# wenyuqing/panacea

Measured on AMD Instinct MI355X. Metric: denoising steps/s (6-view x 8-frame 256x512), higher is better.
Workload: dtype f16; 1 GPU; BASELINE config 3: Panacea+ stage-2 UNet+ControlNet, CFG 2 x 8 frames, 6 views, latent 32x384, hint 256x3072, Euler/LegacyDDPM 50-step schedule; precision=precise: split(stream,gn_stt,ff_out,stem,gn_head,gnt)+e4m3-lo, parallelism=single, graph=False, streams=2, hoisted_step_invariants=False, fused_step_tail=True

## Files before the change

### include/panacea_hip.h

```cpp
#ifndef PANACEA_HIP_H
#define PANACEA_HIP_H

#include <stdint.h>

#ifdef __cplusplus
extern "C" {
#endif

#define PNC_OK 0
#define PNC_EINVAL (-1)
#define PNC_EALIGN (-2)
#define PNC_EABI (-3)

const char* pnc_version(void);
#define PNC_ABI_VERSION 8
int pnc_abi_version(void);
const char* pnc_build_digest(void);

enum {
    PNC_OPT_GEMM_TAIL_SPLIT = 0,
    PNC_OPT_GEMM_TILE = 1,
    PNC_OPT_ATTN_VARIANT = 2,
    PNC_OPT_ATTN_DMA = 3,
    PNC_OPT_GEMM_FUSE_LN = 4,
    PNC_OPT_GEMM_GROUP_M = 5,
    PNC_OPT_STENCIL_TILES = 6,
    PNC_OPT_GEMM_PERSIST = 7,
    PNC_OPT_ATTN_DEFER_MAX = 8,
    PNC_OPT_GEMM_GN_STATS = 9,
    PNC_OPT_GEMM_STAGGER = 10,
    PNC_OPT_ATTN_SUM_TRIGGER = 11,
    PNC_OPT_COUNT = 12
};
int pnc_set_option(int option, int value);

enum { PNC_A_PLAIN = 0, PNC_A_CONV3X3 = 1, PNC_A_CONV1D_T = 2 };
enum { PNC_LO_F16 = 0, PNC_LO_E4M3 = 1 };
enum { PNC_ACT_NONE = 0, PNC_ACT_SILU = 1, PNC_ACT_GELU = 2  };

typedef struct PncGemmParams {
    const void* A;
    const void* W;
    int32_t M, N, K;
    int32_t lda;
    int32_t a_mode;
    int32_t Cin, Hin, Win, Hout, Wout, stride, upsample;
    int32_t T, Npix;
    const float* bias;
    const float* rowbias;
    int32_t rb_rows, rb_mod;
    const float* res1; int32_t ldr1;
    const float* res2; int32_t ldr2;
    float*  out32;  int32_t ldc32;
    void*   out16;  int32_t ldc16;
    void*   out16t; int32_t ldt; int32_t t_rows; int64_t t_gstride;
    int32_t n_split;
    int32_t act;
    int32_t geglu;
    float*  ws;
    int64_t ws_floats;
    int32_t conv_pad_br;
    int32_t struct_bytes;
    const void* A_lo;
    void* out16_lo;
    int32_t ldw;
    float ln_eps;
    const float* ln_gamma;
    const float* ln_beta;
    void* ln_out16;
    int32_t ldln;
    int32_t a_lo_fmt;
    int32_t out_lo_fmt;
    int32_t ldw_lo;
    const void* W_lo;
    int32_t w_lo_exp;
    int32_t t_halo;
    int64_t x_halo_off;
    float* gn_part;
} PncGemmParams;

int pnc_gemm_f16(const PncGemmParams* p, void* stream);
int pnc_gemm_wsplit_f16(const PncGemmParams* p, const void* W_lo16, void* stream);
int pnc_gemm_fuses_layernorm(const PncGemmParams* p);
int64_t pnc_gemm_workspace_floats(const PncGemmParams* p);

// ... 147 lines not shown
```

### panacea_amd/csrc/attn.hip

```cpp
#include "common.h"
#include "attn_check.h"

namespace {

constexpr int KT = 64;

__device__ __forceinline__ int kperm(int i) { return 16 * ((i >> 2) & 1) + 4 * (i >> 3) + (i & 3); }

__device__ __attribute__((aligned(16))) half_t g_attn_zero_chunk[8];

template <int NW, int QB, bool DMA>
__global__ __launch_bounds__(64 * NW, (NW == 4 && QB == 2 && DMA) ? 2 : 1) void attn_views_kernel(const PncAttnParams p, const int wv_shift,
                                                                                          const float defer_thr, const int dma_mode,
                                                                                          const float sum_lim) {
    constexpr int QT = NW * QB * 32;
    constexpr int ROWS_PER_IT = NW * 8;
    constexpr int ST_IT = 64 / ROWS_PER_IT;
    constexpr int NST = DMA ? 3 : 2;
    __shared__ __attribute__((aligned(16))) char smem[NST * 2 * KT * 128];
    const half_t* __restrict__ Q = reinterpret_cast<const half_t*>(p.q);
    const half_t* __restrict__ K = reinterpret_cast<const half_t*>(p.k);
    const half_t* __restrict__ VT = reinterpret_cast<const half_t*>(p.vt);
    half_t* __restrict__ O = reinterpret_cast<half_t*>(p.o);
    auto seg_view = [&](int id, const half_t*& Kb, const half_t*& Vb) -> int {
// ... 561 lines not shown
    half_t* slab = sv[wv];
    {
        half_t* d = slab + vr * TW_ROW + 32 * (vp >> 1) + 8 * (vp & 1);
        *reinterpret_cast<half4v*>(d) = half4v{v0[0], v0[1], v0[2], v0[3]};
        *reinterpret_cast<half4v*>(d + 16) = half4v{v0[4], v0[5], v0[6], v0[7]};
        *reinterpret_cast<half4v*>(d + 4) = half4v{v1[0], v1[1], v1[2], v1[3]};
        *reinterpret_cast<half4v*>(d + 20) = half4v{v1[4], v1[5], v1[6], v1[7]};
    }
    f32x4 s = {0.0f, 0.0f, 0.0f, 0.0f};
    s = __builtin_amdgcn_mfma_f32_16x16x32_f16(k0, q0, s, 0, 0, 0);
    s = __builtin_amdgcn_mfma_f32_16x16x32_f16(k1, q1, s, 0, 0, 0);
    const float c = scale * 1.44269504088896340736f;
    float sc[4];
    float mx = -INFINITY;
#pragma unroll
    for (int i = 0; i < 4; ++i) {
        sc[i] = (4 * g + i < T) ? s[i] * c : -INFINITY;
        mx = fmaxf(mx, sc[i]);
    }
    mx = fmaxf(mx, __shfl_xor(mx, 16, 64));
    mx = fmaxf(mx, __shfl_xor(mx, 32, 64));
    float l = 0.0f;
    half4v ph;
#pragma unroll
    for (int i = 0; i < 4; ++i) {
        const float p = (4 * g + i < T) ? exp2f(sc[i] - mx) : 0.0f;
        l += p;
        ph[i] = (half_t)p;
    }
    l += __shfl_xor(l, 16, 64);
    l += __shfl_xor(l, 32, 64);
    const float inv = 1.0f / l;
    __builtin_amdgcn_wave_barrier();
    typedef __fp16 tr_half4v __attribute__((__vector_size__(4 * sizeof(__fp16))));
    typedef __attribute__((address_space(3))) tr_half4v lds_half4v;
    const half_t* tr = slab + (4 * g + ((lane >> 2) & 3)) * TW_ROW + 4 * (lane & 3);
#pragma unroll
    for (int e = 0; e < 2; ++e) {
        f32x4 acc[2];
#pragma unroll
        for (int h = 0; h < 2; ++h) {
            const half4v vt = __builtin_bit_cast(half4v, __builtin_amdgcn_ds_read_tr16_b64_v4f16((lds_half4v*)(tr + 32 * e + 16 * h)));
            acc[h] = __builtin_amdgcn_mfma_f32_16x16x16f16(vt, ph, f32x4{0.0f, 0.0f, 0.0f, 0.0f}, 0, 0, 0);
        }
        if (r < T) {
            half8v o;
#pragma unroll
            for (int i = 0; i < 4; ++i) { o[i] = (half_t)(acc[0][i] * inv); o[4 + i] = (half_t)(acc[1][i] * inv); }
            *reinterpret_cast<half8v*>(O + row * ldo + col + 32 * e + 8 * g) = o;
        }
    }
}

constexpr int TEXT_HG = 5;

int attn_views_check(const PncAttnParams* pp) {
    if (!pp) return PNC_EINVAL;
    const PncAttnParams& p = *pp;
    if (!p.q || !p.k || !p.vt || !p.o) return PNC_EINVAL;
    if (!pnc_attn::views_ok(p)) return PNC_EINVAL;
    if (p.ldq % 8 || p.ldk % 8 || p.ldo % 4) return PNC_EALIGN;
    if ((((uintptr_t)p.q | (uintptr_t)p.k | (uintptr_t)p.vt) & 15) || ((uintptr_t)p.o & 7)) return PNC_EALIGN;
    if (!pnc_attn::counts_ok(p)) return PNC_EINVAL;
    if (p.causal != 0 && p.causal != 1) return PNC_EINVAL;
    for (int v = 0; v < p.views; ++v) {
        if (!pnc_attn::nseg_ok(p, v)) return PNC_EINVAL;
        for (int s = 0; s < p.nseg[v]; ++s) {
            const int id = p.seg[v][s];
            if (id == -1 || id == p.kv_views) {
                const int side = id < 0 ? 0 : 1;
                if (!p.k_halo[side] || !p.vt_halo[side]) return PNC_EINVAL;
                if (((uintptr_t)p.k_halo[side] | (uintptr_t)p.vt_halo[side]) & 15) return PNC_EALIGN;
            } else if (id < 0 || id > p.kv_views) {
                return PNC_EINVAL;
            }
        }
    }
    return PNC_OK;
}

bool attn_text_dispatch(const PncAttnParams& p) {
    const bool text_ok = p.views == 1 && p.kv_views == 1 && p.nseg[0] == 1 && p.seg[0][0] == 0 && !p.causal && p.kvH * p.kvW <= 96 &&
                         ((p.kvH * p.kvW) & 7) == 0 && p.kv_valid > 64 && p.kv_valid <= 96 && (p.ldvt & 7) == 0 &&
                         (p.vt_gstride & 7) == 0 && (p.ldk & 7) == 0;
    const int force = pnc_get_option(PNC_OPT_ATTN_VARIANT);
    const int Nq = p.H * (p.W / p.views);
    const int nhg = (p.heads + TEXT_HG - 1) / TEXT_HG;
    const bool big_enough = (long)((Nq + 127) / 128) * nhg >= 16;
    const int dopt = pnc_get_option(PNC_OPT_ATTN_DMA);
    return text_ok && (force == 43 || (force == 0 && big_enough)) && (dopt & 3) != 0 && !(dopt & 4);
}

int views_variant(const PncAttnParams& p, int Nq, int force) {
    if (force >= 41) return force;
    if (p.kv_valid * 2 <= 256) {
        return Nq >= 256 ? 42 : 41;
    }
    if (Nq >= 512) return force == 1 ? 82 : 42;
    if (Nq >= 256) return 81;
    return 41;
}

struct ViewsArgs { int wv_shift; float defer_thr; int dma_mode; bool dma; float sum_lim; };
ViewsArgs views_args(const PncAttnParams& p) {
    const int kvWv = p.kvW / p.kv_views, dma_mode = pnc_get_option(PNC_OPT_ATTN_DMA) & 3;
    const int dopt = pnc_get_option(PNC_OPT_ATTN_DEFER_MAX), sopt = pnc_get_option(PNC_OPT_ATTN_SUM_TRIGGER);
// ... 5 lines not shown

template <int NW, int QB>
void launch_views(const PncAttnParams& p, const ViewsArgs& a, hipStream_t st) {
    constexpr int QTILE = 32 * NW * QB;
    const int Nq = p.H * (p.W / p.views);
    const dim3 grid(((Nq + QTILE - 1) / QTILE) * p.views * p.groups * p.heads), block(64 * NW);
    hipLaunchKernelGGL((a.dma ? attn_views_kernel<NW, QB, true> : attn_views_kernel<NW, QB, false>), grid, block, 0, st, p, a.wv_shift, a.defer_thr,
                       a.dma_mode, a.sum_lim);
}

template <typename... Sig, typename... Tail>
void launch_temporal(void (*kernel)(Sig...), int64_t nwork, void* stream, const void* q, int ldq, const void* k, int ldk,
                     const void* v, int ldv, void* o, int ldo, Tail... tail) {
    hipLaunchKernelGGL(kernel, dim3((unsigned)((nwork + 3) / 4)), dim3(256), 0, reinterpret_cast<hipStream_t>(stream), f16p(q), ldq,
                       f16p(k), ldk, f16p(v), ldv, f16p(o), ldo, tail...);
}

}

extern "C" int pnc_attn_uses_text_kernel(const PncAttnParams* pp) {
    return attn_views_check(pp) == PNC_OK && attn_text_dispatch(*pp) ? 1 : 0;
}

extern "C" int pnc_attn_views_f16(const PncAttnParams* pp, void* stream) {
    const int rc = attn_views_check(pp);
    if (rc != PNC_OK) return rc;
    const PncAttnParams& p = *pp;
    hipStream_t st = reinterpret_cast<hipStream_t>(stream);
    const int Nq = p.H * (p.W / p.views);
    if (attn_text_dispatch(p)) {
        const int nhg = (p.heads + TEXT_HG - 1) / TEXT_HG;
        const dim3 grid((unsigned)((long)((Nq + 127) / 128) * nhg * p.groups));
        hipLaunchKernelGGL((attn_text_kernel<TEXT_HG>), grid, dim3(256), 0, st, p, nhg);
        return pnc_launch_status();
    }
    const ViewsArgs a = views_args(p);
    switch (views_variant(p, Nq, pnc_get_option(PNC_OPT_ATTN_VARIANT))) {
        case 42: launch_views<4, 2>(p, a, st); break;
        case 82: launch_views<8, 2>(p, a, st); break;
        case 81: launch_views<8, 1>(p, a, st); break;
        default: launch_views<4, 1>(p, a, st);
    }
    return pnc_launch_status();
}

extern "C" int pnc_attn_temporal_f16(const void* q, int ldq, const void* k, int ldk,
                                     const void* v, int ldv, void* o, int ldo,
                                     int B, int T, int Npix, int heads, float scale, void* stream) {
    if (!q || !k || !v || !o) return PNC_EINVAL;
    if (T < 1 || T > 16 || B < 1 || Npix < 1 || heads < 1) return PNC_EINVAL;
    if (ldq % 8 || ldk % 8 || ldv % 8 || ldo % 8) return PNC_EALIGN;
    if (((uintptr_t)q | (uintptr_t)k | (uintptr_t)v | (uintptr_t)o) & 15) return PNC_EALIGN;
    const bool wide = T > 8;
    const int ppw = wide ? 1 : 8 / T;
    const int64_t nwork = (int64_t)B * ((Npix + ppw - 1) / ppw) * heads;
    if (wide && nwork > 0x7fffffff) return PNC_EINVAL;
    if (wide) launch_temporal(attn_temporal_wide_kernel, nwork, stream, q, ldq, k, ldk, v, ldv, o, ldo, T, Npix, heads, scale, (unsigned)nwork);
    else launch_temporal(attn_temporal_kernel, nwork, stream, q, ldq, k, ldk, v, ldv, o, ldo, B, T, Npix, heads, scale, ppw, nwork);
    return pnc_launch_status();
}
```

### panacea_amd/csrc/misc.hip

```cpp
#include "common.h"
#include <atomic>

namespace {

constexpr int SM_MAXM = 16;

__global__ __launch_bounds__(256) void linear_smallm_kernel(const float* __restrict__ a, int lda,
                                                            const half_t* __restrict__ W,
                                                            const half_t* __restrict__ W_lo,
                                                            const float* __restrict__ bias,
                                                            float* __restrict__ out, int ldo, int M, int N,
                                                            int K, int silu_in, int silu_out) {
    const int lane = threadIdx.x & 63;
    const int n = blockIdx.x * 4 + (threadIdx.x >> 6);
    if (n >= N) return;
    float acc[SM_MAXM];
#pragma unroll
    for (int m = 0; m < SM_MAXM; ++m) acc[m] = 0.0f;
    for (int k0 = lane * 8; k0 < K; k0 += 64 * 8) {
        const half8v w = *reinterpret_cast<const half8v*>(W + (int64_t)n * K + k0);
        float wf[8];
#pragma unroll
        for (int e = 0; e < 8; ++e) wf[e] = (float)w[e];
        if (W_lo) {
// ... 331 lines not shown
        ok = p.out_aux && p.n_hist >= 0 && p.n_hist <= 3;
        for (int k = 0; ok && k < p.n_hist; ++k) ok = p.hist[k] != nullptr;
        break;
    default: return PNC_EINVAL;
    }
    for (int k = 0; ok && k < nv; ++k) ok = p.v[k] != nullptr;
    if (!ok) return PNC_EINVAL;
    return launch_1d(skip ? cfg_sampler_step_kernel<true> : cfg_sampler_step_kernel<false>, (int64_t)p.T * p.Npix, stream, p,
                     c_skip);
}

int cfg_euler_step_launch(const float* eps_tok, int ld, int T, int Npix, int C, int cfg, float scale, const float* x,
                          const float* c_out, const float* sigma, const float* sigma_next, float* x_next, const float* c_skip,
                          bool skip, void* stream) {
    PncSamplerStepParams p = {};
    p.struct_bytes = (int32_t)sizeof(PncSamplerStepParams);
    p.mode = PNC_SAMPLER_HEUN1;
    p.eps_tok = eps_tok, p.ld = ld, p.T = T, p.Npix = Npix, p.C = C, p.cfg = cfg, p.scale = scale;
    p.x = x, p.c_out = c_out, p.v[0] = sigma, p.v[1] = sigma_next, p.out = x_next;
    return cfg_sampler_step_launch(&p, c_skip, skip, true, stream);
}

}

extern "C" int pnc_cfg_euler_step(const float* eps_tok, int ld, int T, int Npix, int C, int cfg, float scale,
                                  const float* x, const float* c_out, const float* sigma, const float* sigma_next,
                                  float* x_next, void* stream) {
    return cfg_euler_step_launch(eps_tok, ld, T, Npix, C, cfg, scale, x, c_out, sigma, sigma_next, x_next, nullptr, false, stream);
}

extern "C" int pnc_cfg_euler_step_skip(const float* eps_tok, int ld, int T, int Npix, int C, int cfg, float scale,
                                       const float* x, const float* c_skip, const float* c_out, const float* sigma,
                                       const float* sigma_next, float* x_next, void* stream) {
    return cfg_euler_step_launch(eps_tok, ld, T, Npix, C, cfg, scale, x, c_out, sigma, sigma_next, x_next, c_skip, true, stream);
}

extern "C" int pnc_cfg_sampler_step(const PncSamplerStepParams* pp, void* stream) {
    return cfg_sampler_step_launch(pp, nullptr, false, false, stream);
}

extern "C" int pnc_cfg_sampler_step_skip(const PncSamplerStepParams* pp, const float* c_skip, void* stream) {
    return cfg_sampler_step_launch(pp, c_skip, true, false, stream);
}

extern "C" const char* pnc_version(void) { return "panacea_hip 0.4.0 gfx950"; }
#ifndef PNC_BUILD_DIGEST
#define PNC_BUILD_DIGEST "unstamped"
#endif
static const char k_build_digest[] = "pnc-build-digest:" PNC_BUILD_DIGEST;
extern "C" const char* pnc_build_digest(void) { return k_build_digest + 17; }

static std::atomic<int> g_options[PNC_OPT_COUNT] = {{1}, {0}, {0}, {1}, {1}, {0}, {1}, {3}, {8}, {1}, {4}, {12}};

int pnc_get_option(int option) { return g_options[option].load(std::memory_order_relaxed); }

extern "C" int pnc_set_option(int option, int value) {
    if (option < 0 || option >= PNC_OPT_COUNT) return PNC_EINVAL;
    return g_options[option].exchange(value, std::memory_order_relaxed);
}

extern "C" int pnc_linear_smallm_split(const float* a, int lda, const void* W, const void* W_lo, const float* bias,
                                       float* out, int ldo, int M, int N, int K, int silu_in, int silu_out,
                                       void* stream) {
    if (!a || !W || !out || M < 1 || M > SM_MAXM || N < 1 || K < 8) return PNC_EINVAL;
    if (K % 8 || lda % 4) return PNC_EINVAL;
    if (((uintptr_t)a | (uintptr_t)W | (uintptr_t)W_lo) & 15) return PNC_EALIGN;
    return launch_1d(linear_smallm_kernel, (int64_t)N * 64, stream, a, lda, f16p(W), f16p(W_lo), bias, out, ldo, M, N, K, silu_in,
                     silu_out);
}

extern "C" int pnc_linear_smallm(const float* a, int lda, const void* W, const float* bias,
                                 float* out, int ldo, int M, int N, int K, int silu_in, int silu_out,
                                 void* stream) {
    return pnc_linear_smallm_split(a, lda, W, nullptr, bias, out, ldo, M, N, K, silu_in, silu_out, stream);
}

extern "C" int pnc_linear_smallm_segments(const float* a, int lda, const void* W, const float* bias, float* out, int M,
                                          int m0, int Mtot, int N, int K, const int32_t* seg_start, int nseg, int silu_in,
                                          int silu_out, void* stream) {
    return pnc_linear_smallm_segments_split(a, lda, W, nullptr, bias, out, M, m0, Mtot, N, K, seg_start, nseg, silu_in, silu_out, stream);
}

extern "C" int pnc_linear_smallm_segments_split(const float* a, int lda, const void* W, const void* W_lo, const float* bias,
                                                float* out, int M, int m0, int Mtot, int N, int K, const int32_t* seg_start,
                                                int nseg, int silu_in, int silu_out, void* stream) {
    if (!a || !W || !out || !seg_start || M < 1 || M > SM_MAXM || m0 < 0 || m0 + M > Mtot || N < 1 || K < 8) return PNC_EINVAL;
    if (K % 8 || lda % 4 || nseg < 1 || nseg > PNC_SMALLM_MAX_SEGS) return PNC_EINVAL;
    if (((uintptr_t)a | (uintptr_t)W | (uintptr_t)W_lo) & 15) return PNC_EALIGN;
    SmallmSegs segs;
    segs.nseg = nseg;
    if (seg_start[0] != 0 || seg_start[nseg] != N) return PNC_EINVAL;
    for (int i = 0; i <= nseg; ++i) {
        if (seg_start[i] % SEG_NC || (i > 0 && seg_start[i] <= seg_start[i - 1])) return PNC_EINVAL;
        segs.start[i] = seg_start[i];
    }
    return launch_1d(linear_smallm_seg_kernel, (int64_t)(N / SEG_NC) * 64, stream, a, lda, f16p(W), f16p(W_lo), bias, out, M, m0, Mtot,
                     N, K, silu_in, silu_out, segs);
}

template <typename TS>
static int timestep_embedding(const TS* t, int F, int dim, const float* freqs, float* out, void* stream) {
    if (!t || !out || !freqs || F < 1 || dim < 2) return PNC_EINVAL;
    return launch_1d(timestep_embedding_kernel<TS>, F * (dim / 2), stream, t, F, dim, freqs, out);
}

extern "C" int pnc_timestep_embedding(const int64_t* t, int F, int dim, const float* freqs,
                                      float* out, void* stream) {
    return timestep_embedding(t, F, dim, freqs, out, stream);
}
// ... 122 lines not shown
```

### panacea_amd/csrc/norm.hip

```cpp
#include "common.h"
#include <type_traits>

namespace {

constexpr int GROUPS = 32;


__device__ __forceinline__ int gn_wave_pixels(int np, int w) { return np > w ? (np - w + 3) >> 2 : 0; }

template <int J>
__device__ __forceinline__ bool gn_reduce_records(float* sm, int Cs, int cpg, int ng, int np, const float2 (&pv)[J],
                                                  const f32x4 (&sum)[J], const f32x4 (&sq)[J], float& n, float& mean, float& m2) {
    const int tid = threadIdx.x, lane = tid & 63, wave = tid >> 6;
    const int CVs = Cs >> 2;
    float* mine = sm + wave * Cs;
    float* s_gmean = sm + 4 * Cs;
    const float nw = (float)gn_wave_pixels(np, wave);
    const float inw = nw > 0.0f ? 1.0f / nw : 0.0f;
    const float icpg = 1.0f / (float)cpg;
    f32x4 m[J];
#pragma unroll
    for (int j = 0; j < J; ++j) {
        const int cv = lane + j * 64;
#pragma unroll
// ... 394 lines not shown
        if (row0 + r >= M) break;
        const float rs = rsqrtf(rstd[r] + eps);
        half_t* yr = y + (row0 + r) * ldy;
#pragma unroll
        for (int j = 0; j < J; ++j) {
            const int cv = lane + j * 64;
            if (cv < CV) {
                half4v h;
                float o[4];
#pragma unroll
                for (int e = 0; e < 4; ++e) { o[e] = fmaf((v[r][j][e] - mean[r]) * rs, g[j][e], b[j][e]); h[e] = (half_t)o[e]; }
                *reinterpret_cast<half4v*>(yr + cv * 4) = h;
                if (ylo) *reinterpret_cast<half4v*>(ylo + (row0 + r) * ldy + cv * 4) = lo_plane4(o, h);
            }
        }
    }
}

__global__ __launch_bounds__(256) void gn_combine_kernel(const float* __restrict__ in, int parts, int F, int nchunk,
                                                         float* __restrict__ out) {
    __shared__ float s_pn[8 * GROUPS], s_pm[8 * GROUPS], s_p2[8 * GROUPS];
    const int f = blockIdx.x, tid = threadIdx.x;
    const int g = tid & 31, part = tid >> 5;
    const int nrec = parts * nchunk;
    float n = 0.0f, mean = 0.0f, m2 = 0.0f;
    for (int r = part; r < nrec; r += 8) {
        const int s = r / nchunk, c = r - s * nchunk;
        const float* q = in + ((((int64_t)s * F + f) * nchunk + c) * GROUPS + g) * 3;
        const float nb = q[0], mb = q[1], m2b = q[2];
        const float nt = n + nb, d = mb - mean;
        const float w = nb / fmaxf(nt, 1.0f);
        mean = fmaf(d, w, mean);
        m2 += m2b + d * d * (n * w);
        n = nt;
    }
    s_pn[part * GROUPS + g] = n; s_pm[part * GROUPS + g] = mean; s_p2[part * GROUPS + g] = m2;
    __syncthreads();
    if (tid < GROUPS) {
        float tn = 0.0f, tm = 0.0f, t2 = 0.0f;
        for (int k = 0; k < 8; ++k) {
            const float nb = s_pn[k * GROUPS + tid], mb = s_pm[k * GROUPS + tid], m2b = s_p2[k * GROUPS + tid];
            const float nt = tn + nb, d = mb - tm;
            const float w = nb / fmaxf(nt, 1.0f);
            tm = fmaf(d, w, tm);
            t2 += m2b + d * d * (tn * w);
            tn = nt;
        }
        float* o = out + ((int64_t)f * nchunk * GROUPS + tid) * 3;
        o[0] = tn; o[1] = tm; o[2] = t2;
    }
    for (int i = GROUPS * 3 + tid; i < nchunk * GROUPS * 3; i += 256) out[(int64_t)f * nchunk * GROUPS * 3 + i] = 0.0f;
}

template <int J>
__global__ __launch_bounds__(256) void concat_add_stats_kernel(const float* __restrict__ a, int C1, const float* __restrict__ s,
                                                               const float* __restrict__ c, int C2, int Npix, int ppc,
                                                               float* __restrict__ out32, half_t* __restrict__ out16,
                                                               void* __restrict__ out16_lo, int lo_fmt, float* __restrict__ partial) {
    extern __shared__ __attribute__((aligned(16))) float sm[];
    const int f = blockIdx.y, chunk = blockIdx.x, nchunk = gridDim.x, S = gridDim.z, z = blockIdx.z;
    const int tid = threadIdx.x, lane = tid & 63, wave = tid >> 6;
    const int C = C1 + C2, cpg = C / GROUPS;
    const int Cs = C / S, c0 = z * Cs, CVs = Cs >> 2, gps = GROUPS / S;
    const int p0 = chunk * ppc;
    const int p1 = min(Npix, p0 + ppc);
    f32x4 sum[J], sq[J];
    float2 pv[J];
    const f32x4 zz = {0.0f, 0.0f, 0.0f, 0.0f};
#pragma unroll
    for (int j = 0; j < J; ++j) { sum[j] = zz; sq[j] = zz; pv[j] = make_float2(0.0f, 0.0f); }
#pragma unroll 2
    for (int pix = p0 + wave; pix < p1; pix += 4) {
        const int64_t m = (int64_t)f * Npix + pix;
        f32x4 v[J];
#pragma unroll
        for (int j = 0; j < J; ++j) {
            const int cv = lane + j * 64, ch = c0 + cv * 4;
            v[j] = zz;
            if (cv < CVs) {
                if (ch < C1) {
                    v[j] = *reinterpret_cast<const f32x4*>(a + m * C1 + ch);
                } else {
                    v[j] = *reinterpret_cast<const f32x4*>(s + m * C2 + (ch - C1));
                    if (c) v[j] += *reinterpret_cast<const f32x4*>(c + m * C2 + (ch - C1));
                }
            }
        }
        const bool first = pix == p0 + wave;
#pragma unroll
        for (int j = 0; j < J; ++j) {
            const int cv = lane + j * 64, ch = c0 + cv * 4;
            if (cv < CVs) {
                if (out32) *reinterpret_cast<f32x4*>(out32 + m * C + ch) = v[j];
                if (out16) {
                    half4v h = {(half_t)v[j][0], (half_t)v[j][1], (half_t)v[j][2], (half_t)v[j][3]};
                    *reinterpret_cast<half4v*>(out16 + m * C + ch) = h;
                    if (out16_lo) {
                        const float o[4] = {v[j][0], v[j][1], v[j][2], v[j][3]};
                        store_lo4(out16_lo, lo_fmt, m * C + ch, o, h);
                    }
                }
            }
            if (first) pv[j] = make_float2(v[j][0], v[j][2]);
            const f32x4 d = v[j] - f32x4{pv[j].x, pv[j].x, pv[j].y, pv[j].y};
            sum[j] += d;
#pragma unroll
            for (int e = 0; e < 4; ++e) sq[j][e] = fmaf(d[e], d[e], sq[j][e]);
        }
    }
    float n, mean, m2;
    if (gn_reduce_records<J>(sm, Cs, cpg, gps, p1 - p0, pv, sum, sq, n, mean, m2)) {
// ... 24 lines not shown
    return {PB, (unsigned)(((int64_t)B * Npix + PB - 1) / PB), ((size_t)PB * (C / 2) * 2 + (size_t)PB * GROUPS * 2) * sizeof(float)};
}

template <int MODE>
int launch_gn_temporal(int T, void* stream, const float* x, int B, int Npix, int C, const float* gamma, const float* beta, float eps,
                       void* y16, void* y16_lo, int lo_fmt, float* stats, int T_total, int t_pad) {
    if (((uintptr_t)x | (uintptr_t)gamma | (uintptr_t)beta) & 15) return PNC_EALIGN;
    if (((uintptr_t)y16 | (uintptr_t)y16_lo | (uintptr_t)stats) & 7) return PNC_EALIGN;
    const GnTemporalGeom g = gn_temporal_geom(B, Npix, C);
    auto launch = [&](auto frames) {
        constexpr int TT = decltype(frames)::value;
        hipLaunchKernelGGL((gn_temporal_kernel<TT, MODE>), dim3(g.blocks), dim3(TT <= 8 ? 256 : 512), g.lds, reinterpret_cast<hipStream_t>(stream),
                           x, B, Npix, C, gamma, beta, eps, f16p(y16), y16_lo, lo_fmt, g.PB, stats, T_total, t_pad);
    };
    switch (T) {
        case 1: launch(int_c<1>{}); break; case 2: launch(int_c<2>{}); break; case 3: launch(int_c<3>{}); break; case 4: launch(int_c<4>{}); break;
        case 5: launch(int_c<5>{}); break; case 6: launch(int_c<6>{}); break; case 7: launch(int_c<7>{}); break; case 8: launch(int_c<8>{}); break;
        case 9: launch(int_c<9>{}); break; case 10: launch(int_c<10>{}); break; case 11: launch(int_c<11>{}); break; case 12: launch(int_c<12>{}); break;
        case 13: launch(int_c<13>{}); break; case 14: launch(int_c<14>{}); break; case 15: launch(int_c<15>{}); break; case 16: launch(int_c<16>{}); break;
    }
    return pnc_launch_status();
}

}

extern "C" int pnc_groupnorm_stats(const float* x, int ldx, int F, int Npix, int C,
                                   int pix_per_chunk, float* partial, void* stream) {
    if (!x || !partial || F < 1 || Npix < 1 || pix_per_chunk < 1) return PNC_EINVAL;
    if (C % 64 || C > GN_MAXC || ldx % 4) return PNC_EINVAL;
    if ((uintptr_t)x & 15) return PNC_EALIGN;
    const int nchunk = (Npix + pix_per_chunk - 1) / pix_per_chunk;
    const size_t lds = ((size_t)4 * C + GROUPS) * sizeof(float);
    hipStream_t st = reinterpret_cast<hipStream_t>(stream);
    dispatch_j(vectors_per_lane(C), [&](auto j) {
        hipLaunchKernelGGL(gn_stats_kernel<decltype(j)::value>, dim3(nchunk, F), dim3(256), lds, st, x, ldx, Npix, C, pix_per_chunk, partial);
    });
    return pnc_launch_status();
}

extern "C" int pnc_concat_add_stats(const float* a, int C1, const float* s, const float* c, int C2, int F, int Npix, int pix_per_chunk,
                                    float* out32, void* out16, void* out16_lo, int lo_fmt, float* partial, void* stream) {
    if (!a || !s || !partial || F < 1 || Npix < 1 || pix_per_chunk < 1 || C1 % 4 || C2 % 4 || C1 < 4 || C2 < 4) return PNC_EINVAL;
    if (lo_fmt != PNC_LO_F16 && lo_fmt != PNC_LO_E4M3) return PNC_EINVAL;
    if ((!out32 && !out16) || (out16_lo && !out16)) return PNC_EINVAL;
    const int C = C1 + C2;
    if (C % 64 || C > GN_MAXC) return PNC_EINVAL;
    if (((uintptr_t)a | (uintptr_t)s | (uintptr_t)c | (uintptr_t)out32) & 15) return PNC_EALIGN;
    const int nchunk = (Npix + pix_per_chunk - 1) / pix_per_chunk;
    int S = 1;
    while (S < 8 && vectors_per_lane(C / S) > 3 && (C / (2 * S)) % 4 == 0) S *= 2;
    if (vectors_per_lane(C / S) > 3) return PNC_EINVAL;
    const size_t lds = ((size_t)4 * (C / S) + GROUPS) * sizeof(float);
    hipStream_t st = reinterpret_cast<hipStream_t>(stream);
    dispatch_j<3>(vectors_per_lane(C / S), [&](auto j) {
        hipLaunchKernelGGL(concat_add_stats_kernel<decltype(j)::value>, dim3(nchunk, F, S), dim3(256), lds, st, a, C1, s, c, C2, Npix, pix_per_chunk,
                           out32, f16p(out16), out16_lo, lo_fmt, partial);
    });
    return pnc_launch_status();
}

extern "C" int pnc_groupnorm_apply(const float* x, int ldx, int F, int Npix, int C,
                                   int pix_per_chunk, const float* partial,
                                   const float* gamma, const float* beta, float eps, int silu,
                                   void* y16, int ldy, void* y16_lo, int lo_fmt, int n_records, void* stream) {
    if (!x || !partial || !gamma || !beta || !y16 || F < 1 || Npix < 1 || pix_per_chunk < 1 || n_records < 0) return PNC_EINVAL;
    if (lo_fmt != PNC_LO_F16 && lo_fmt != PNC_LO_E4M3) return PNC_EINVAL;
    if (C % 64 || C > GN_MAXC || ldx % 4 || ldy % 4) return PNC_EINVAL;
    if (((uintptr_t)x & 15) || (((uintptr_t)y16 | (uintptr_t)y16_lo) & 7)) return PNC_EALIGN;
    const int nchunk = (Npix + pix_per_chunk - 1) / pix_per_chunk;
    const size_t lds = ((size_t)(2 * C > 24 * GROUPS ? 2 * C : 24 * GROUPS) + 2 * GROUPS) * sizeof(float);
    hipStream_t st = reinterpret_cast<hipStream_t>(stream);
    dispatch_j(vectors_per_lane(C), [&](auto j) {
        hipLaunchKernelGGL(gn_apply_kernel<decltype(j)::value>, dim3(nchunk, F), dim3(256), lds, st, x, ldx, Npix, C, pix_per_chunk, partial,
                           gamma, beta, eps, silu, f16p(y16), ldy, y16_lo, lo_fmt, n_records > 0 ? n_records : nchunk);
    });
    return pnc_launch_status();
}

extern "C" int pnc_groupnorm_combine(const float* in, int parts, int F, int nchunk, float* out, void* stream) {
    if (!in || !out || parts < 1 || F < 1 || nchunk < 1) return PNC_EINVAL;
    hipLaunchKernelGGL(gn_combine_kernel, dim3(F), dim3(256), 0, reinterpret_cast<hipStream_t>(stream), in, parts, F, nchunk, out);
    return pnc_launch_status();
}

extern "C" int pnc_groupnorm_temporal_silu(const float* x, int B, int T, int Npix, int C,
                                           const float* gamma, const float* beta, float eps,
                                           void* y16, void* y16_lo, int lo_fmt, void* stream) {
    if (!x || !gamma || !beta || !y16 || B < 1 || Npix < 1) return PNC_EINVAL;
    if (lo_fmt != PNC_LO_F16 && lo_fmt != PNC_LO_E4M3) return PNC_EINVAL;
    if (C % 64 || C > 2048 || T < 1 || T > 16) return PNC_EINVAL;
    return launch_gn_temporal<0>(T, stream, x, B, Npix, C, gamma, beta, eps, y16, y16_lo, lo_fmt, nullptr, T, 0);
}

extern "C" int pnc_groupnorm_temporal_part(const float* x, int B, int T, int Npix, int C,
                                           const float* gamma, const float* beta, float eps,
                                           float* stats, int mode, int T_total,
                                           void* y16, void* y16_lo, int lo_fmt, int t_pad, void* stream) {
    if (!x || !stats || B < 1 || Npix < 1 || (mode != 1 && mode != 2)) return PNC_EINVAL;
    if (C % 64 || C > 2048 || T < 1 || T > 16 || T_total < T || (t_pad != 0 && t_pad != 1)) return PNC_EINVAL;
    if (mode == 2 && (!gamma || !beta || !y16 || (lo_fmt != PNC_LO_F16 && lo_fmt != PNC_LO_E4M3))) return PNC_EINVAL;
    return (mode == 1 ? launch_gn_temporal<1> : launch_gn_temporal<2>)(T, stream, x, B, Npix, C, gamma, beta, eps, y16, y16_lo, lo_fmt, stats, T_total, t_pad);
}

extern "C" int pnc_layernorm(const float* x, int ldx, int M, int C,
                             const float* gamma, const float* beta, float eps,
                             void* y16, int ldy, void* y16_lo, void* stream) {
    if (!x || !gamma || !beta || !y16 || M < 1) return PNC_EINVAL;
    if (C % 4 || C > 4 * 64 * 12 || C < 4 || ldx % 4 || ldy % 4) return PNC_EINVAL;
    if (((uintptr_t)x | (uintptr_t)gamma | (uintptr_t)beta) & 15) return PNC_EALIGN;
// ... 12 lines not shown
```

### panacea_amd/hip.py

```python
from __future__ import annotations

import ctypes as C
import re
from pathlib import Path
from typing import Optional

import torch

PKG = Path(__file__).resolve().parent
LIB_PATH = PKG / "lib" / "libpanacea_hip.so"
HEADER = PKG.parent / "include" / "panacea_hip.h"

A_PLAIN, A_CONV3X3, A_CONV1D_T = 0, 1, 2
ACT_NONE, ACT_SILU, ACT_GELU = 0, 1, 2
ABI_VERSION = 8
LO_F16, LO_E4M3 = 0, 1
LO_DTYPE = {LO_F16: torch.float16, LO_E4M3: torch.uint8}


def lo_fmt(t: Optional[torch.Tensor]) -> int:
    if t is None or t.dtype == torch.float16:
        return LO_F16
    if t.dtype == torch.uint8:
        return LO_E4M3
# ... 125 lines not shown

def header_symbols() -> list[str]:
    txt = HEADER.read_text()
    txt = re.sub(r"/\*.*?\*/", "", txt, flags=re.S)
    return sorted(set(re.findall(r"\b(pnc_[a-z0-9_]+)\s*\(", txt)))


def load():
    global _lib
    if _lib is not None:
        return _lib
    import os
    global LIB_PATH
    if os.environ.get("PANACEA_HIP_LIB"):
        LIB_PATH = Path(os.environ["PANACEA_HIP_LIB"])
    if not LIB_PATH.exists():
        raise HipLibraryError(
            f"{LIB_PATH} is missing: the HIP extension is the only compute path of panacea_amd. "
            "Build it with `python -m panacea_amd.build` (hipcc --offload-arch=gfx950).")
    try:
        lib = C.CDLL(str(LIB_PATH))
    except OSError as e:
        raise HipLibraryError(f"cannot load {LIB_PATH}: {e}") from e
    if not os.environ.get("PANACEA_HIP_LIB"):
        from . import build as _build
        try:
            lib.pnc_build_digest.restype = C.c_char_p
            have = lib.pnc_build_digest().decode()
        except AttributeError:
            have = "(a library older than pnc_build_digest)"
        if _build.CSRC.exists() and have != _build._digest():
            raise HipLibraryError(f"{LIB_PATH} was built from other sources ({have[:12]}) than panacea_amd/csrc holds now "
                                  f"({_build._digest()[:12]}); rebuild it with `python -m panacea_amd.build`")
    for name, (res, args) in _SIGNATURES.items():
        try:
            fn = getattr(lib, name)
        except AttributeError as e:
            raise HipLibraryError(f"{LIB_PATH} does not export {name}; rebuild the extension") from e
        fn.restype = res
        fn.argtypes = args
    if lib.pnc_abi_version() != ABI_VERSION:
        raise HipLibraryError(f"{LIB_PATH} implements C-ABI version {lib.pnc_abi_version()}, this binding needs "
                              f"{ABI_VERSION}; rebuild the extension (`python -m panacea_amd.build --force`)")
    _lib = lib
    return lib


OPT_GEMM_TAIL_SPLIT, OPT_GEMM_TILE, OPT_ATTN_VARIANT, OPT_ATTN_DMA, OPT_GEMM_FUSE_LN, OPT_GEMM_GROUP_M, OPT_STENCIL_TILES = 0, 1, 2, 3, 4, 5, 6
OPT_GEMM_PERSIST = 7
OPT_ATTN_DEFER_MAX = 8
OPT_GEMM_GN_STATS = 9
OPT_GEMM_STAGGER = 10
OPT_ATTN_SUM_TRIGGER = 11


def build_digest() -> str:
    return load().pnc_build_digest().decode()


def set_option(option: int, value: int) -> int:
    if not 0 <= option <= OPT_ATTN_SUM_TRIGGER:
        raise PncError(f"unknown library option {option}")
    return load().pnc_set_option(option, value)


CU_MASK_PATTERNS = {
    "even-odd": ([0x55555555] * 8, [0xAAAAAAAA] * 8),
    "nibbles": ([0x0F0F0F0F] * 8, [0xF0F0F0F0] * 8),
    "halves": ([0xFFFFFFFF] * 4 + [0] * 4, [0] * 4 + [0xFFFFFFFF] * 4),
}


def masked_stream(words) -> "torch.cuda.Stream":
    rt = None
    for line in open("/proc/self/maps"):
        if "libamdhip64" in line:
            rt = C.CDLL(line.split()[-1])
            break
    if rt is None:
        raise PncError("the HIP runtime is not loaded")
    rt.hipExtStreamCreateWithCUMask.argtypes = [C.POINTER(C.c_void_p), C.c_uint32, C.POINTER(C.c_uint32)]
    rt.hipExtStreamCreateWithCUMask.restype = C.c_int
    st = C.c_void_p()
    arr = (C.c_uint32 * len(words))(*words)
    rc = rt.hipExtStreamCreateWithCUMask(C.byref(st), C.c_uint32(len(words)), arr)
    if rc != 0:
        raise PncError(f"hipExtStreamCreateWithCUMask failed with {rc}")
    return torch.cuda.ExternalStream(st.value)


class Profiler:

    def __init__(self):
        self.records = []

    def summary(self) -> dict:
        torch.cuda.synchronize()
        out = {}
        for fam, e0, e1, fl, by in self.records:
            d = out.setdefault(fam, dict(launches=0, ms=0.0, flops=0.0, bytes=0.0))
            d["launches"] += 1
            d["ms"] += e0.elapsed_time(e1)
            d["flops"] += fl
            d["bytes"] += by
        return out


_PROF: Optional[Profiler] = None


def set_profiler(p: Optional[Profiler]):
    global _PROF
    _PROF = p

# ... 379 lines not shown
```

Measured before the change: 6.504 steps/s.

## Pack two pixels per wave in temporal attention and batch concat-stats loads

Adds a packed temporal-attention kernel that puts 16/T pixels' frames into one 16-row MFMA tile per wave, masking cross-pixel scores, and makes it the default for T<=8. It also rewrites the concat+add+GroupNorm-stats kernel to issue loads for several pixel rows before computing, to hide memory latency. The old paths stay behind a new legacy option bitmask. The packed kernel uses an extra hi/lo split of the probability matrix for precision, which doubles the PV MFMAs, and relies on float-based pixel index division.

```diff
diff --git a/include/panacea_hip.h b/include/panacea_hip.h
--- a/include/panacea_hip.h
+++ b/include/panacea_hip.h
@@ -30,7 +30,8 @@
     PNC_OPT_GEMM_GN_STATS = 9,
     PNC_OPT_GEMM_STAGGER = 10,
     PNC_OPT_ATTN_SUM_TRIGGER = 11,
-    PNC_OPT_COUNT = 12
+    PNC_OPT_COUNT = 12,
+    PNC_OPT_STREAM_LEGACY = 64
 };
 int pnc_set_option(int option, int value);
 
diff --git a/panacea_amd/csrc/attn.hip b/panacea_amd/csrc/attn.hip
--- a/panacea_amd/csrc/attn.hip
+++ b/panacea_amd/csrc/attn.hip
@@ -637,6 +637,98 @@
     }
 }
 
+__global__ __launch_bounds__(256) void attn_temporal_packed_kernel(
+    const half_t* __restrict__ Q, int ldq, const half_t* __restrict__ Kp, int ldk,
+    const half_t* __restrict__ Vp, int ldv, half_t* __restrict__ O, int ldo,
+    int T, int Npix, int heads, float scale, int P, int groups_per_b, unsigned nwork) {
+    __shared__ __attribute__((aligned(16))) half_t sv[4][16 * TW_ROW];
+    const int lane = threadIdx.x & 63, wv = threadIdx.x >> 6;
+    const unsigned w = blockIdx.x * 4u + (unsigned)wv;
+    if (w >= nwork) return;
+    const unsigned bg = w / (unsigned)heads;
+    const int head = (int)(w - bg * (unsigned)heads);
+    const unsigned b = bg / (unsigned)groups_per_b;
+    const int pix0 = (int)(bg - b * (unsigned)groups_per_b) * P;
+    const int nrow = min(P, Npix - pix0) * T;
+    const int64_t base = (int64_t)b * T * Npix + pix0;
+    const float iT = 1.0f / (float)T;
+    auto pixel_of = [iT](int x) { return (int)(((float)x + 0.5f) * iT); };
+    const int col = head * 64;
+    const int r = lane & 15, g = lane >> 4;
+    const bool rok = r < nrow;
+    const int rps = pixel_of(r);
+    const int64_t row = base + (rok ? (int64_t)(r - rps * T) * Npix + rps : 0);
+    const half_t* qp = Q + row * ldq + col + 16 * g;
+    const half_t* kp = Kp + row * ldk + col + 16 * g;
+    const half8v q0 = *reinterpret_cast<const half8v*>(qp), q1 = *reinterpret_cast<const half8v*>(qp + 8);
+    const half8v k0 = *reinterpret_cast<const half8v*>(kp), k1 = *reinterpret_cast<const half8v*>(kp + 8);
+    const int vr = lane >> 2, vp = lane & 3;
+    const bool vok = vr < nrow;
+    const int vps = pixel_of(vr);
+    const half_t* vptr = Vp + (base + (vok ? (int64_t)(vr - vps * T) * Npix + vps : 0)) * ldv + col + 16 * vp;
+    half8v v0 = *reinterpret_cast<const half8v*>(vptr), v1 = *reinterpret_cast<const half8v*>(vptr + 8);
+    if (!vok) {
+#pragma unroll
+        for (int i = 0; i < 8; ++i) { v0[i] = (half_t)0; v1[i] = (half_t)0; }
+    }
+    half_t* slab = sv[wv];
+    {
+        half_t* d = slab + vr * TW_ROW + 32 * (vp >> 1) + 8 * (vp & 1);
+        *reinterpret_cast<half4v*>(d) = half4v{v0[0], v0[1], v0[2], v0[3]};
+        *reinterpret_cast<half4v*>(d + 16) = half4v{v0[4], v0[5], v0[6], v0[7]};
+        *reinterpret_cast<half4v*>(d + 4) = half4v{v1[0], v1[1], v1[2], v1[3]};
+        *reinterpret_cast<half4v*>(d + 20) = half4v{v1[4], v1[5], v1[6], v1[7]};
+    }
+    f32x4 s = {0.0f, 0.0f, 0.0f, 0.0f};
+    s = __builtin_amdgcn_mfma_f32_16x16x32_f16(k0, q0, s, 0, 0, 0);
+    s = __builtin_amdgcn_mfma_f32_16x16x32_f16(k1, q1, s, 0, 0, 0);
+    const float c = scale * 1.44269504088896340736f;
+    float sc[4];
+    bool kok[4];
+    float mx = -INFINITY;
+#pragma unroll
+    for (int i = 0; i < 4; ++i) {
+        const int kr = 4 * g + i;
+        kok[i] = rok && kr < nrow && pixel_of(kr) == rps;
+        sc[i] = kok[i] ? s[i] * c : -INFINITY;
+        mx = fmaxf(mx, sc[i]);
+    }
+    mx = fmaxf(mx, __shfl_xor(mx, 16, 64));
+    mx = fmaxf(mx, __shfl_xor(mx, 32, 64));
+    float l = 0.0f;
+    half4v ph, pl;
+#pragma unroll
+    for (int i = 0; i < 4; ++i) {
+        const float p = kok[i] ? exp2f(sc[i] - mx) : 0.0f;
+        l += p;
+        ph[i] = (half_t)p;
+        pl[i] = (half_t)(p - (float)ph[i]);
+    }
+    l += __shfl_xor(l, 16, 64);
+    l += __shfl_xor(l, 32, 64);
+    const float inv = rok ? 1.0f / l : 0.0f;
+    __builtin_amdgcn_wave_barrier();
+    typedef __fp16 tr_half4v __attribute__((__vector_size__(4 * sizeof(__fp16))));
+    typedef __attribute__((address_space(3))) tr_half4v lds_half4v;
+    const half_t* tr = slab + (4 * g + ((lane >> 2) & 3)) * TW_ROW + 4 * (lane & 3);
+#pragma unroll
+    for (int e = 0; e < 2; ++e) {
+        f32x4 acc[2];
+#pragma unroll
+        for (int h = 0; h < 2; ++h) {
+            const half4v vt = __builtin_bit_cast(half4v, __builtin_amdgcn_ds_read_tr16_b64_v4f16((lds_half4v*)(tr + 32 * e + 16 * h)));
+            acc[h] = __builtin_amdgcn_mfma_f32_16x16x16f16(vt, pl, f32x4{0.0f, 0.0f, 0.0f, 0.0f}, 0, 0, 0);
+            acc[h] = __builtin_amdgcn_mfma_f32_16x16x16f16(vt, ph, acc[h], 0, 0, 0);
+        }
+        if (rok) {
+            half8v o;
+#pragma unroll
+            for (int i = 0; i < 4; ++i) { o[i] = (half_t)(acc[0][i] * inv); o[4 + i] = (half_t)(acc[1][i] * inv); }
+            *reinterpret_cast<half8v*>(O + row * ldo + col + 32 * e + 8 * g) = o;
+        }
+    }
+}
+
 constexpr int TEXT_HG = 5;
 
 int attn_views_check(const PncAttnParams* pp) {
@@ -748,6 +840,14 @@
     if (ldq % 8 || ldk % 8 || ldv % 8 || ldo % 8) return PNC_EALIGN;
     if (((uintptr_t)q | (uintptr_t)k | (uintptr_t)v | (uintptr_t)o) & 15) return PNC_EALIGN;
     const bool wide = T > 8;
+    if (!wide && !(pnc_get_option(PNC_OPT_STREAM_LEGACY) & 2)) {
+        const int P = 16 / T, gpb = (Npix + P - 1) / P;
+        const int64_t nw = (int64_t)B * gpb * heads;
+        if (nw <= 0x7fffffff) {
+            launch_temporal(attn_temporal_packed_kernel, nw, stream, q, ldq, k, ldk, v, ldv, o, ldo, T, Npix, heads, scale, P, gpb, (unsigned)nw);
+            return pnc_launch_status();
+        }
+    }
     const int ppw = wide ? 1 : 8 / T;
     const int64_t nwork = (int64_t)B * ((Npix + ppw - 1) / ppw) * heads;
     if (wide && nwork > 0x7fffffff) return PNC_EINVAL;
diff --git a/panacea_amd/csrc/misc.hip b/panacea_amd/csrc/misc.hip
--- a/panacea_amd/csrc/misc.hip
+++ b/panacea_amd/csrc/misc.hip
@@ -407,9 +407,15 @@
 
 static std::atomic<int> g_options[PNC_OPT_COUNT] = {{1}, {0}, {0}, {1}, {1}, {0}, {1}, {3}, {8}, {1}, {4}, {12}};
 
-int pnc_get_option(int option) { return g_options[option].load(std::memory_order_relaxed); }
+static std::atomic<int> g_stream_legacy{0};
+
+int pnc_get_option(int option) {
+    if (option == PNC_OPT_STREAM_LEGACY) return g_stream_legacy.load(std::memory_order_relaxed);
+    return g_options[option].load(std::memory_order_relaxed);
+}
 
 extern "C" int pnc_set_option(int option, int value) {
+    if (option == PNC_OPT_STREAM_LEGACY) return g_stream_legacy.exchange(value, std::memory_order_relaxed);
     if (option < 0 || option >= PNC_OPT_COUNT) return PNC_EINVAL;
     return g_options[option].exchange(value, std::memory_order_relaxed);
 }
diff --git a/panacea_amd/csrc/norm.hip b/panacea_amd/csrc/norm.hip
--- a/panacea_amd/csrc/norm.hip
+++ b/panacea_amd/csrc/norm.hip
@@ -470,11 +470,87 @@
     for (int i = GROUPS * 3 + tid; i < nchunk * GROUPS * 3; i += 256) out[(int64_t)f * nchunk * GROUPS * 3 + i] = 0.0f;
 }
 
+constexpr int CONCAT_R = 4;
 template <int J>
 __global__ __launch_bounds__(256) void concat_add_stats_kernel(const float* __restrict__ a, int C1, const float* __restrict__ s,
                                                                const float* __restrict__ c, int C2, int Npix, int ppc,
                                                                float* __restrict__ out32, half_t* __restrict__ out16,
                                                                void* __restrict__ out16_lo, int lo_fmt, float* __restrict__ partial) {
+    extern __shared__ __attribute__((aligned(16))) float sm[];
+    const int f = blockIdx.y, chunk = blockIdx.x, nchunk = gridDim.x, S = gridDim.z, z = blockIdx.z;
+    const int tid = threadIdx.x, lane = tid & 63, wave = tid >> 6;
+    const int C = C1 + C2, cpg = C / GROUPS;
+    const int Cs = C / S, c0 = z * Cs, CVs = Cs >> 2, gps = GROUPS / S;
+    const int p0 = chunk * ppc;
+    const int p1 = min(Npix, p0 + ppc);
+    constexpr int R = CONCAT_R;
+    f32x4 sum[J], sq[J];
+    float2 pv[J];
+    const f32x4 zz = {0.0f, 0.0f, 0.0f, 0.0f};
+#pragma unroll
+    for (int j = 0; j < J; ++j) { sum[j] = zz; sq[j] = zz; pv[j] = make_float2(0.0f, 0.0f); }
+    for (int pix0 = p0 + wave; pix0 < p1; pix0 += 4 * R) {
+        f32x4 v[R][J], u[R][J];
+#pragma unroll
+        for (int rr = 0; rr < R; ++rr) {
+            const int pix = pix0 + 4 * rr;
+            const int64_t m = (int64_t)f * Npix + pix;
+#pragma unroll
+            for (int j = 0; j < J; ++j) {
+                const int cv = lane + j * 64, ch = c0 + cv * 4;
+                v[rr][j] = zz; u[rr][j] = zz;
+                if (cv < CVs && pix < p1) {
+                    if (ch < C1) {
+                        v[rr][j] = *reinterpret_cast<const f32x4*>(a + m * C1 + ch);
+                    } else {
+                        v[rr][j] = *reinterpret_cast<const f32x4*>(s + m * C2 + (ch - C1));
+                        if (c) u[rr][j] = *reinterpret_cast<const f32x4*>(c + m * C2 + (ch - C1));
+                    }
+                }
+            }
+        }
+#pragma unroll
+        for (int rr = 0; rr < R; ++rr) {
+            const int pix = pix0 + 4 * rr;
+            if (pix >= p1) break;
+            const int64_t m = (int64_t)f * Npix + pix;
+            const bool first = pix == p0 + wave;
+#pragma unroll
+            for (int j = 0; j < J; ++j) {
+                const int cv = lane + j * 64, ch = c0 + cv * 4;
+                f32x4 x = v[rr][j];
+                if (c && ch >= C1) x += u[rr][j];
+                if (cv < CVs) {
+                    if (out32) *reinterpret_cast<f32x4*>(out32 + m * C + ch) = x;
+                    if (out16) {
+                        half4v h = {(half_t)x[0], (half_t)x[1], (half_t)x[2], (half_t)x[3]};
+                        *reinterpret_cast<half4v*>(out16 + m * C + ch) = h;
+                        if (out16_lo) {
+                            const float o[4] = {x[0], x[1], x[2], x[3]};
+                            store_lo4(out16_lo, lo_fmt, m * C + ch, o, h);
+                        }
+                    }
+                }
+                if (first) pv[j] = make_float2(x[0], x[2]);
+                const f32x4 d = x - f32x4{pv[j].x, pv[j].x, pv[j].y, pv[j].y};
+                sum[j] += d;
+#pragma unroll
+                for (int e = 0; e < 4; ++e) sq[j][e] = fmaf(d[e], d[e], sq[j][e]);
+            }
+        }
+    }
+    float n, mean, m2;
+    if (gn_reduce_records<J>(sm, Cs, cpg, gps, p1 - p0, pv, sum, sq, n, mean, m2)) {
+        float* o = partial + ((int64_t)(f * nchunk + chunk) * GROUPS + z * gps + tid) * 3;
+        o[0] = n; o[1] = mean; o[2] = m2;
+    }
+}
+
+template <int J>
+__global__ __launch_bounds__(256) void concat_add_stats_rowwise_kernel(const float* __restrict__ a, int C1, const float* __restrict__ s,
+                                                                       const float* __restrict__ c, int C2, int Npix, int ppc,
+                                                                       float* __restrict__ out32, half_t* __restrict__ out16,
+                                                                       void* __restrict__ out16_lo, int lo_fmt, float* __restrict__ partial) {
     extern __shared__ __attribute__((aligned(16))) float sm[];
     const int f = blockIdx.y, chunk = blockIdx.x, nchunk = gridDim.x, S = gridDim.z, z = blockIdx.z;
     const int tid = threadIdx.x, lane = tid & 63, wave = tid >> 6;
@@ -605,9 +681,11 @@
     if (vectors_per_lane(C / S) > 3) return PNC_EINVAL;
     const size_t lds = ((size_t)4 * (C / S) + GROUPS) * sizeof(float);
     hipStream_t st = reinterpret_cast<hipStream_t>(stream);
+    const bool rowwise = pnc_get_option(PNC_OPT_STREAM_LEGACY) & 1;
     dispatch_j<3>(vectors_per_lane(C / S), [&](auto j) {
-        hipLaunchKernelGGL(concat_add_stats_kernel<decltype(j)::value>, dim3(nchunk, F, S), dim3(256), lds, st, a, C1, s, c, C2, Npix, pix_per_chunk,
-                           out32, f16p(out16), out16_lo, lo_fmt, partial);
+        constexpr int J = decltype(j)::value;
+        hipLaunchKernelGGL(rowwise ? concat_add_stats_rowwise_kernel<J> : concat_add_stats_kernel<J>, dim3(nchunk, F, S), dim3(256), lds, st, a, C1,
+                           s, c, C2, Npix, pix_per_chunk, out32, f16p(out16), out16_lo, lo_fmt, partial);
     });
     return pnc_launch_status();
 }
diff --git a/panacea_amd/hip.py b/panacea_amd/hip.py
--- a/panacea_amd/hip.py
+++ b/panacea_amd/hip.py
@@ -201,6 +201,7 @@
 OPT_GEMM_GN_STATS = 9
 OPT_GEMM_STAGGER = 10
 OPT_ATTN_SUM_TRIGGER = 11
+OPT_STREAM_LEGACY = 64
 
 
 def build_digest() -> str:
@@ -208,7 +209,7 @@
 
 
 def set_option(option: int, value: int) -> int:
-    if not 0 <= option <= OPT_ATTN_SUM_TRIGGER:
+    if not 0 <= option <= OPT_ATTN_SUM_TRIGGER and option != OPT_STREAM_LEGACY:
         raise PncError(f"unknown library option {option}")
     return load().pnc_set_option(option, value)
 
```

Measured after the change: 6.522 steps/s, median of 6. No clear change (+0.3%).
